# ychalier/transflow

Hardware: AMD Instinct MI355X
Metric: frames/sec (Farneback+remap) (higher is better)
Workload: dtype f32; 1 GPU; 4k: one clip of T=256 3840x2160 uint8 frames sharded over the ranks (rank r owns pairs shard_range(255, r, 1) + a one-frame halo), Farneback pyr_scale=0.5 levels=5 winsize=15 iterations=3 poly_n=5 poly_sigma=1.2 flags=0, BACKWARD post_process, moveref layer (reset random p=0.5 through a float mask, u drawn on the GPU), 1 RGB pixmap source, render; clip_frames=256, equal_batches=False

## Files before the change

### transflow_amd/csrc/common.h

```cpp
#pragma once
#include <hip/hip_runtime.h>

#include <cstdarg>
#include <cstdint>
#include <cstdio>
#include <cstdlib>
#include <string>
#include <vector>

#include "../../include/tfhip.h"

#define TF_API extern "C" __attribute__((visibility("default")))

namespace tf {

int set_error(int code, const char *fmt, ...) __attribute__((format(printf, 2, 3)));
hipStream_t stream();
hipStream_t main_stream();
int side_stream(int which, hipStream_t *out);
int ensure_init();

enum Opt { OPT_FB_FUSED = 0, OPT_FB_FUSE_MIN_PX, OPT_FB_NO_SHARE, OPT_FB_NO_OVERLAP, OPT_REMAP_PX, OPT_REMAP_NO_PACK, OPT_REMAP_KEEP_RGBA,
           OPT_PROF_LEVELS, OPT_FB_EXACT_SUMS, OPT_FB_CHAIN, OPT_FB_SEGS, OPT_REMAP_QUAD, OPT_JD_PAR_SUB_BYTES,
           OPT_JD_PAR_GROUP_SUBS, OPT_JD_PAR_STAGED, OPT_REMAP_LEAN, OPT_COUNT };
long option(Opt which);

#ifdef TF_EXPERIMENT
inline long tune(const char *env, long dflt)
{
    const char *v = getenv(env);
    return v ? atol(v) : dflt;
}
inline const char *tune_str(const char *env) { return getenv(env); }
#else
constexpr long tune(const char *, long dflt) { return dflt; }
constexpr const char *tune_str(const char *) { return nullptr; }
#endif

struct StreamScope {
    explicit StreamScope(hipStream_t s);
    ~StreamScope();
    hipStream_t prev;
};

#define TF_HIP(expr)                                                                              \
    do {                                                                                          \
        hipError_t _e = (expr);                                                                   \
        if (_e != hipSuccess)                                                                     \
            return tf::set_error(TF_ERR_HIP, "%s failed: %s (%s:%d)", #expr, hipGetErrorString(_e), \
                                 __FILE__, __LINE__);                                             \
    } while (0)

#define TF_TRY(expr)        \
    do {                    \
        int _rc = (expr);   \
        if (_rc != TF_OK)   \
            return _rc;     \
    } while (0)

#define TF_REQUIRE(cond, ...)                         \
    do {                                              \
        if (!(cond))                                  \
            return tf::set_error(TF_ERR_ARG, __VA_ARGS__); \
    } while (0)

struct ProfScope {
    explicit ProfScope(const char *name);
    ~ProfScope();
    const char *name;
    hipEvent_t a, b;
};
bool prof_enabled();

template <typename K, typename... Args>
inline int launch(const char *name, K kernel, dim3 grid, dim3 block, size_t smem, Args... args)
{
    if (grid.x == 0 || grid.y == 0 || grid.z == 0)
        return TF_OK;
    {
        ProfScope ps(name);
        hipLaunchKernelGGL(kernel, grid, block, smem, stream(), args...);
    }
    hipError_t e = hipGetLastError();
    if (e != hipSuccess)
        return set_error(TF_ERR_HIP, "launch %s failed: %s", name, hipGetErrorString(e));
    return TF_OK;
}

struct DevBuf {
    void *p = nullptr;
    size_t bytes = 0;
    bool borrowed = false;
    DevBuf() = default;
    DevBuf(const DevBuf &) = delete;
    DevBuf &operator=(const DevBuf &) = delete;
    ~DevBuf() { release(); }
    int alloc(size_t n);
    void borrow(void *ptr, size_t n);
    void release();
    template <typename T> T *as() const { return reinterpret_cast<T *>(p); }
};

struct PinnedBuf {
    void *p = nullptr;
    PinnedBuf() = default;
    PinnedBuf(const PinnedBuf &) = delete;
    PinnedBuf &operator=(const PinnedBuf &) = delete;
    ~PinnedBuf() { release(); }
    int alloc(size_t n);
    void release();
    template <typename T> T *as() const { return reinterpret_cast<T *>(p); }
};

struct Event {
    hipEvent_t e = nullptr;
    Event() = default;
    Event(const Event &) = delete;
    Event &operator=(const Event &) = delete;
    ~Event() { release(); }
    int create();
    void release();
    operator hipEvent_t() const { return e; }
};

inline unsigned cdiv(size_t a, size_t b) { return (unsigned)((a + b - 1) / b); }

struct FastDiv {
    uint32_t m;
    int s1, s2;
};
inline FastDiv fast_div_setup(uint32_t d)
{
    int s = 0;
    while ((1ull << s) < d)
        s++;
    FastDiv f;
    f.m = (uint32_t)(((1ull << 32) * ((1ull << s) - d)) / d + 1);
    f.s1 = s < 1 ? s : 1;
    f.s2 = s > 1 ? s - 1 : 0;
    return f;
}
__device__ __forceinline__ uint32_t fast_div(uint32_t t, FastDiv f)
{
    const uint32_t hi = __umulhi(t, f.m);
    return (((t - hi) >> f.s1) + hi) >> f.s2;
}

__device__ __forceinline__ float clip_nan(float v, float lo, float hi) { return v != v ? v : fminf(fmaxf(v, lo), hi); }

__device__ __forceinline__ int clampi(int v, int lo, int hi) { return v < lo ? lo : (v > hi ? hi : v); }

struct PpLabels {
    const char *clip, *fwd_scatter, *fwd_resolve, *ops;
};
constexpr PpLabels PP_FB{"pp_clip", "pp_fwd_scatter", "pp_fwd_resolve", "pp_ops"};
constexpr PpLabels PP_FLOW{"flow_pp_clip", "flow_pp_fwd_scatter", "flow_pp_fwd_resolve", "flow_pp_ops"};
int pp_ops(float2 *flow, int W, int H, int n_ops, const tf_flow_op *ops, const float *mask_dev, const PpLabels &lb);
int pp_scatter(const float2 *flow, int W, int H, int *winner, const PpLabels &lb);
int pp_direction(void *flow, bool wide, int W, int H, int direction, int *winner, const PpLabels &lb);

}
```

### transflow_amd/csrc/fb_pyramid.hip

```cpp
#include "fb_common.h"

namespace {

#ifndef TF_PX_TH
#define TF_PX_TH 16
#endif
constexpr int PX_TW = 64, PX_TH = TF_PX_TH;

__global__ void k_polyexp(const float *__restrict__ img, float *__restrict__ R, int Wk, int Hk, PolyConst pc)
{
    extern __shared__ float s_mem[];
    const int n = pc.n;
    const int LW = PX_TW + 2 * n;
    const int LH = PX_TH + 2 * n;
    float *sI = s_mem;
    float *sT = s_mem + LH * LW;
    const int pi = blockIdx.z;
    const size_t Nk = (size_t)Wk * Hk;
    const float *src = img + (size_t)pi * Nk;
    const int x0 = blockIdx.x * PX_TW, y0 = blockIdx.y * PX_TH;
    for (int idx = threadIdx.x; idx < LH * LW; idx += blockDim.x) {
        int ry = idx / LW, cx = idx % LW;
        int y = clampi(y0 - n + ry, 0, Hk - 1), x = clampi(x0 - n + cx, 0, Wk - 1);
        sI[idx] = src[(size_t)y * Wk + x];
    }
    __syncthreads();
    for (int idx = threadIdx.x; idx < PX_TH * LW; idx += blockDim.x) {
        int ty = idx / LW, cx = idx % LW;
        int y = y0 + ty;
        const float c = sI[(ty + n) * LW + cx];
        float t0 = c * pc.g[0], t1 = 0.f, t2 = 0.f;
        for (int k = 1; k <= n; k++) {
            int ya = max(y - k, 0), yb = min(y + k, Hk - 1);
            float a = sI[(ya - y0 + n) * LW + cx];
            float b = sI[(yb - y0 + n) * LW + cx];
            float p = a + b;
            t0 = t0 + pc.g[k] * p;
            t1 = t1 + pc.xg[k] * (b - a);
            t2 = t2 + pc.xxg[k] * p;
        }
        if (y >= Hk) {
            t0 = t1 = t2 = 0.f;
        }
        sT[(0 * PX_TH + ty) * LW + cx] = t0;
        sT[(1 * PX_TH + ty) * LW + cx] = t1;
        sT[(2 * PX_TH + ty) * LW + cx] = t2;
    }
    __syncthreads();
    float *dst = R + (size_t)pi * 5 * Nk;
    for (int idx = threadIdx.x; idx < PX_TH * PX_TW; idx += blockDim.x) {
        int ty = idx / PX_TW, cx = idx % PX_TW;
        int x = x0 + cx, y = y0 + ty;
        if (x >= Wk || y >= Hk)
            continue;
        const float *T0 = sT + (0 * PX_TH + ty) * LW + cx + n;
        const float *T1 = sT + (1 * PX_TH + ty) * LW + cx + n;
        const float *T2 = sT + (2 * PX_TH + ty) * LW + cx + n;
        float g0 = pc.g[0];
        double b1 = T0[0] * g0, b2 = 0, b3 = T1[0] * g0, b4 = 0, b5 = T2[0] * g0, b6 = 0;
        for (int k = 1; k <= n; k++) {
            double tg = T0[k] + T0[-k];
            g0 = pc.g[k];
            b1 = __builtin_fma(tg, (double)g0, b1);
            b4 = __builtin_fma(tg, (double)pc.xxg[k], b4);
            b2 += (T0[k] - T0[-k]) * pc.xg[k];
            b3 += (T1[k] + T1[-k]) * g0;
            b6 += (T1[k] - T1[-k]) * pc.xg[k];
            b5 += (T2[k] + T2[-k]) * g0;
        }
        size_t o = (size_t)y * Wk + x;
        const float v[5] = {(float)(b3 * pc.ig11), (float)(b2 * pc.ig11), (float)(b1 * pc.ig03 + b5 * pc.ig33),
                            (float)(b1 * pc.ig03 + b4 * pc.ig33), (float)(b6 * pc.ig55)};
        r_store_px(dst, Nk, o, v);
    }
}

typedef float float2w __attribute__((ext_vector_type(2), aligned(4)));

template <int N>
__device__ __forceinline__ void polyexp_vertical4(const f32x2 (&v)[4 + 2 * N], const PolyConst &pc, float *T0, float *T1,
                                                  float *T2, int LW)
{
#pragma unroll
    for (int q = 0; q < 4; q++) {
        const f32x2 c = v[q + N];
        f32x2 t0 = c * pc.g[0], t1 = {0.f, 0.f}, t2 = {0.f, 0.f};
#pragma unroll
        for (int k = 1; k <= N; k++) {
            const f32x2 a = v[q + N - k], b = v[q + N + k];
            const f32x2 p = a + b;
            t0 = t0 + pc.g[k] * p;
            t1 = t1 + pc.xg[k] * (b - a);
            t2 = t2 + pc.xxg[k] * p;
        }
        *reinterpret_cast<f32x2 *>(T0 + q * LW) = t0;
        *reinterpret_cast<f32x2 *>(T1 + q * LW) = t1;
        *reinterpret_cast<f32x2 *>(T2 + q * LW) = t2;
    }
}

template <int N>
__global__ void __launch_bounds__(256)
k_polyexp_t(const float *__restrict__ img, float *__restrict__ R, int Wk, int Hk, PolyConst pc)
{
    constexpr int TW = PX_TW, TH = PX_TH, LW = TW + 2 * N, LH = TH + 2 * N;
    __shared__ float sI[LH * LW];
    __shared__ float sT[3][TH][LW];
    const int pi = blockIdx.z;
    const size_t Nk = (size_t)Wk * Hk;
    const float *src = img + (size_t)pi * Nk;
    const int x0 = blockIdx.x * TW, y0 = blockIdx.y * TH;
    for (int idx = threadIdx.x; idx < LH * LW; idx += 256) {
        int ry = idx / LW, cx = idx - ry * LW;
        int y = clampi(y0 - N + ry, 0, Hk - 1), x = clampi(x0 - N + cx, 0, Wk - 1);
        sI[idx] = src[(size_t)y * Wk + x];
    }
    __syncthreads();
    static_assert(LW % 2 == 0, "column pairs");
    for (int idx = threadIdx.x; idx < (TH / 4) * (LW / 2); idx += 256) {
        const int g = idx / (LW / 2), cx = 2 * (idx - g * (LW / 2));
        f32x2 v[4 + 2 * N];
#pragma unroll
        for (int j = 0; j < 4 + 2 * N; j++)
            v[j] = *reinterpret_cast<const f32x2 *>(&sI[(4 * g + j) * LW + cx]);
        polyexp_vertical4<N>(v, pc, &sT[0][4 * g][cx], &sT[1][4 * g][cx], &sT[2][4 * g][cx], LW);
    }
    __syncthreads();
    float *dst = R + (size_t)pi * 5 * Nk;
    for (int idx = threadIdx.x; idx < TH * (TW / 2); idx += 256) {
        const int ty = idx / (TW / 2), cp = idx - ty * (TW / 2);
        const int x = x0 + 2 * cp, y = y0 + ty;
        if (x >= Wk || y >= Hk)
            continue;
        float w0[2 + 2 * N], w1[2 + 2 * N], w2[2 + 2 * N];
#pragma unroll
        for (int j = 0; j < 2 + 2 * N; j++) {
            w0[j] = sT[0][ty][2 * cp + j];
            w1[j] = sT[1][ty][2 * cp + j];
            w2[j] = sT[2][ty][2 * cp + j];
        }
        float out[2][5];
#pragma unroll
        for (int q = 0; q < 2; q++) {
            const float *T0 = w0 + q + N, *T1 = w1 + q + N, *T2 = w2 + q + N;
            float g0 = pc.g[0];
            double b1 = T0[0] * g0, b2 = 0, b3 = T1[0] * g0, b4 = 0, b5 = T2[0] * g0, b6 = 0;
#pragma unroll
            for (int k = 1; k <= N; k++) {
                double tg = T0[k] + T0[-k];
                g0 = pc.g[k];
                b1 = __builtin_fma(tg, (double)g0, b1);
                b4 = __builtin_fma(tg, (double)pc.xxg[k], b4);
                b2 += (T0[k] - T0[-k]) * pc.xg[k];
                b3 += (T1[k] + T1[-k]) * g0;
                b6 += (T1[k] - T1[-k]) * pc.xg[k];
                b5 += (T2[k] + T2[-k]) * g0;
            }
            out[q][0] = (float)(b3 * pc.ig11);
            out[q][1] = (float)(b2 * pc.ig11);
            out[q][2] = (float)(b1 * pc.ig03 + b5 * pc.ig33);
            out[q][3] = (float)(b1 * pc.ig03 + b4 * pc.ig33);
            out[q][4] = (float)(b6 * pc.ig55);
        }
        const size_t o = (size_t)y * Wk + x;
        if (x + 1 < Wk)
            r_store_px2(dst, Nk, o, out[0], out[1]);
        else
            r_store_px(dst, Nk, o, out[0]);
    }
}

template <int N, int TW, int TH>
__device__ __forceinline__ void tile_expansion(const float *sI, float (*sT)[TH][TW + 2 * N], int x0, int y0, int xr0,
                                               int yr0, int W, int H, const PolyConst &pc, float *dst, size_t Nk)
{
    constexpr int LW = TW + 2 * N;
    const bool interior = x0 - N >= 0 && x0 + TW - 1 + N <= W - 1 && y0 - N >= 0 && y0 + TH - 1 + N <= H - 1;
    for (int idx = threadIdx.x; idx < (TH / 4) * (LW / 2); idx += 256) {
        const int g = idx / (LW / 2), cx = 2 * (idx - g * (LW / 2));
        f32x2 v[4 + 2 * N];
        if (interior) {
#pragma unroll
            for (int j = 0; j < 4 + 2 * N; j++)
                v[j] = *reinterpret_cast<const f32x2 *>(&sI[(4 * g + j) * LW + cx]);
        } else {
            const int xa = clampi(x0 - N + cx, 0, W - 1) - xr0, xb = clampi(x0 - N + cx + 1, 0, W - 1) - xr0;
#pragma unroll
            for (int j = 0; j < 4 + 2 * N; j++) {
                const float *row = sI + (clampi(y0 - N + 4 * g + j, 0, H - 1) - yr0) * LW;
                v[j] = f32x2{row[xa], row[xb]};
            }
        }
        polyexp_vertical4<N>(v, pc, &sT[0][4 * g][cx], &sT[1][4 * g][cx], &sT[2][4 * g][cx], LW);
    }
    __syncthreads();
    for (int idx = threadIdx.x; idx < TH * (TW / 2); idx += 256) {
        const int ty = idx / (TW / 2), cp = idx - ty * (TW / 2);
        const int x = x0 + 2 * cp, y = y0 + ty;
        if (x >= W || y >= H)
            continue;
        float w0[2 + 2 * N], w1[2 + 2 * N], w2[2 + 2 * N];
#pragma unroll
        for (int j = 0; j < 2 + 2 * N; j++) {
            w0[j] = sT[0][ty][2 * cp + j];
            w1[j] = sT[1][ty][2 * cp + j];
            w2[j] = sT[2][ty][2 * cp + j];
        }
        float out[2][5];
#pragma unroll
        for (int q = 0; q < 2; q++) {
            const float *T0 = w0 + q + N, *T1 = w1 + q + N, *T2 = w2 + q + N;
            float g0 = pc.g[0];
            double b1 = T0[0] * g0, b2 = 0, b3 = T1[0] * g0, b4 = 0, b5 = T2[0] * g0, b6 = 0;
#pragma unroll
            for (int k = 1; k <= N; k++) {
                double tg = T0[k] + T0[-k];
                g0 = pc.g[k];
                b1 = __builtin_fma(tg, (double)g0, b1);
                b4 = __builtin_fma(tg, (double)pc.xxg[k], b4);
                b2 += (T0[k] - T0[-k]) * pc.xg[k];
                b3 += (T1[k] + T1[-k]) * g0;
                b6 += (T1[k] - T1[-k]) * pc.xg[k];
                b5 += (T2[k] + T2[-k]) * g0;
            }
            out[q][0] = (float)(b3 * pc.ig11);
            out[q][1] = (float)(b2 * pc.ig11);
            out[q][2] = (float)(b1 * pc.ig03 + b5 * pc.ig33);
            out[q][3] = (float)(b1 * pc.ig03 + b4 * pc.ig33);
            out[q][4] = (float)(b6 * pc.ig55);
        }
        const size_t o = (size_t)y * W + x;
        if (x + 1 < W)
            r_store_px2(dst, Nk, o, out[0], out[1]);
        else
            r_store_px(dst, Nk, o, out[0]);
    }
}

#ifndef TF_EXP_TH0
#define TF_EXP_TH0 16
#endif
#ifndef TF_EXP_TH1
#define TF_EXP_TH1 24
#endif
template <int N>
__global__ void __launch_bounds__(256)
k_level0_polyexp_t(const uint8_t *__restrict__ frames, const int2 *__restrict__ pairs, float *__restrict__ R, int W,
                   int H, float kc, float k1, PolyConst pc)
{
    constexpr int TW = 64, TH = TF_EXP_TH0, LW = TW + 2 * N, LH = TH + 2 * N;
    constexpr int SW = ((LW + 2 + 3 + 3) + 3) & ~3, SH = LH + 2;
    constexpr int RS = (LW + 3) & ~3;
    static_assert(SW >= RS + 4 + 4 && (SH * SW) % 16 == 0, "a group's three dwords stay inside its staged row; sRow 16-byte aligned");
    constexpr int BYTES_A = SH * SW + SH * RS * 4, BYTES_T = 3 * TH * LW * 4;
    constexpr int BYTES_U = ((BYTES_A > BYTES_T ? BYTES_A : BYTES_T) + 15) & ~15;
    __shared__ __attribute__((aligned(16))) uint8_t s_u[BYTES_U];
    __shared__ float sI[LH * LW];
    uint8_t *sS = s_u;
    float *sRow = reinterpret_cast<float *>(s_u + SH * SW);
    float(*sT)[TH][LW] = reinterpret_cast<float(*)[TH][LW]>(s_u);
    const int pi = blockIdx.z;
    const int2 pr = pairs[pi >> 1];
    const uint8_t *src = frames + (size_t)((pi & 1) ? pr.y : pr.x) * W * H;
    const size_t Nk = (size_t)W * H;
    const int x0 = blockIdx.x * TW, y0 = blockIdx.y * TH;
    const int lane = threadIdx.x & 63, wave = threadIdx.x >> 6;
    const int xr0 = max(x0 - N, 0), xr1 = min(x0 + TW - 1 + N, W - 1);
    const int yr0 = max(y0 - N, 0), yr1 = min(y0 + TH - 1 + N, H - 1);
    const int ny = yr1 - yr0 + 1;
    const int xs = (xr0 - 1) & ~3, off = xr0 - 1 - xs;
    const int ncols = xr1 + 1 - xs + 1;
    const bool dwords = (W & 3) == 0 && xs >= 0 && xs + ((ncols + 3) & ~3) <= W;
    constexpr int U = 8;
    if (dwords) {
        const int nq = (ncols + 3) >> 2;
        for (int c = lane; c < nq; c += 64) {
            for (int j0 = wave; j0 < ny + 2; j0 += 4 * U) {
                uint32_t v[U];
#pragma unroll
                for (int u = 0; u < U; u++) {
                    int ry = j0 + 4 * u;
                    if (ry < ny + 2)
                        v[u] = *reinterpret_cast<const uint32_t *>(src + (size_t)reflect101_near(yr0 - 1 + ry, H) * W + xs + 4 * c);
                }
#pragma unroll
                for (int u = 0; u < U; u++) {
                    int ry = j0 + 4 * u;
                    if (ry < ny + 2)
                        *reinterpret_cast<uint32_t *>(sS + ry * SW + 4 * c) = v[u];
                }
            }
        }
    } else {
        for (int c = lane; c < ncols; c += 64) {
            const int x = reflect101_near(xs + c, W);
            for (int j0 = wave; j0 < ny + 2; j0 += 4 * U) {
                uint8_t v[U];
#pragma unroll
                for (int u = 0; u < U; u++) {
                    int ry = j0 + 4 * u;
                    if (ry < ny + 2)
                        v[u] = src[(size_t)reflect101_near(yr0 - 1 + ry, H) * W + x];
                }
#pragma unroll
                for (int u = 0; u < U; u++) {
                    int ry = j0 + 4 * u;
                    if (ry < ny + 2)
                        sS[ry * SW + c] = v[u];
                }
            }
        }
    }
    __syncthreads();
    for (int idx = threadIdx.x; idx < (ny + 2) * (RS / 4); idx += 256) {
        const int ry = idx / (RS / 4), cx = 4 * (idx - ry * (RS / 4));
        const uint32_t *q = reinterpret_cast<const uint32_t *>(sS + ry * SW + cx);
        const uint32_t d0 = q[0], d1 = q[1], d2 = q[2];
        const uint32_t lo = __builtin_amdgcn_alignbyte(d1, d0, off), hi = __builtin_amdgcn_alignbyte(d2, d1, off);
        const float b0 = (float)(lo & 0xff), b1 = (float)((lo >> 8) & 0xff), b2 = (float)((lo >> 16) & 0xff),
                    b3 = (float)(lo >> 24), b4 = (float)(hi & 0xff), b5 = (float)((hi >> 8) & 0xff);
        float *o = sRow + ry * RS + cx;
        *reinterpret_cast<f32x2 *>(o) = f32x2{b1 * kc + (b0 + b2) * k1, b2 * kc + (b1 + b3) * k1};
        *reinterpret_cast<f32x2 *>(o + 2) = f32x2{b3 * kc + (b2 + b4) * k1, b4 * kc + (b3 + b5) * k1};
    }
    __syncthreads();
    for (int idx = threadIdx.x; idx < ny * (RS / 4); idx += 256) {
        const int ry = idx / (RS / 4), cx = 4 * (idx - ry * (RS / 4));
        const float *c = sRow + (ry + 1) * RS + cx;
        const f32x4 m = *reinterpret_cast<const f32x4 *>(c), dn = *reinterpret_cast<const f32x4 *>(c + RS),
                    up = *reinterpret_cast<const f32x4 *>(c - RS);
        f32x4 v = kc * m;
        v += k1 * (dn + up);
        float *o = sI + ry * LW + cx;
        *reinterpret_cast<f32x2 *>(o) = f32x2{v.x, v.y};
        if (cx + 2 < LW)
            *reinterpret_cast<f32x2 *>(o + 2) = f32x2{v.z, v.w};
    }
    __syncthreads();
    tile_expansion<N, TW, TH>(sI, sT, x0, y0, xr0, yr0, W, H, pc, R + (size_t)pi * 5 * Nk, Nk);
}

template <int N>
__global__ void __launch_bounds__(256)
k_level1_polyexp_t(const uint8_t *__restrict__ frames, const int2 *__restrict__ pairs, float *__restrict__ R, int W,
                   int H, float kc, float k1, PolyConst pc)
{
    constexpr int TW = 64, TH = TF_EXP_TH1, LW = TW + 2 * N, LH = TH + 2 * N;
    constexpr int SW = ((2 * LW + 2 + 3 + 3) + 3) & ~3, SH = 2 * LH + 2;
    constexpr int BYTES_A = SH * SW, BYTES_T = 3 * TH * LW * 4;
    constexpr int BYTES_U = ((BYTES_A > BYTES_T ? BYTES_A : BYTES_T) + 15) & ~15;
    __shared__ __attribute__((aligned(16))) uint8_t s_u[BYTES_U];
    __shared__ float sI[LH * LW];
    uint8_t *sS = s_u;
    float(*sT)[TH][LW] = reinterpret_cast<float(*)[TH][LW]>(s_u);
    const int Wk = W >> 1, Hk = H >> 1;
    const int pi = blockIdx.z;
    const int2 pr = pairs[pi >> 1];
    const uint8_t *src = frames + (size_t)((pi & 1) ? pr.y : pr.x) * W * H;
    const size_t Nk = (size_t)Wk * Hk;
    const int x0 = blockIdx.x * TW, y0 = blockIdx.y * TH;
    const int lane = threadIdx.x & 63, wave = threadIdx.x >> 6;
    const int xr0 = max(x0 - N, 0), xr1 = min(x0 + TW - 1 + N, Wk - 1);
    const int yr0 = max(y0 - N, 0), yr1 = min(y0 + TH - 1 + N, Hk - 1);
    const int ny = yr1 - yr0 + 1;
    const int cfirst = 2 * xr0 - 1, rfirst = 2 * yr0 - 1, nrows = 2 * ny + 2;
    const int xs = cfirst >= 0 ? (cfirst & ~3) : cfirst, off = cfirst - xs;
    const int ncols = 2 * xr1 + 2 - xs + 1;
    const bool dwords = (W & 3) == 0 && xs >= 0 && (xs & 3) == 0 && xs + ((ncols + 3) & ~3) <= W;
    constexpr int U = 8;
    if (dwords) {
        const int nq = (ncols + 3) >> 2;
        for (int c = lane; c < nq; c += 64) {
            for (int j0 = wave; j0 < nrows; j0 += 4 * U) {
                uint32_t v[U];
#pragma unroll
                for (int u = 0; u < U; u++) {
                    int ry = j0 + 4 * u;
                    if (ry < nrows)
                        v[u] = *reinterpret_cast<const uint32_t *>(src + (size_t)reflect101_near(rfirst + ry, H) * W + xs + 4 * c);
                }
#pragma unroll
                for (int u = 0; u < U; u++) {
                    int ry = j0 + 4 * u;
                    if (ry < nrows)
                        *reinterpret_cast<uint32_t *>(sS + ry * SW + 4 * c) = v[u];
                }
            }
        }
    } else {
        for (int c = lane; c < ncols; c += 64) {
            const int x = reflect101_near(xs + c, W);
            for (int j0 = wave; j0 < nrows; j0 += 4 * U) {
                uint8_t v[U];
#pragma unroll
                for (int u = 0; u < U; u++) {
                    int ry = j0 + 4 * u;
                    if (ry < nrows)
                        v[u] = src[(size_t)reflect101_near(rfirst + ry, H) * W + x];
                }
#pragma unroll
                for (int u = 0; u < U; u++) {
                    int ry = j0 + 4 * u;
                    if (ry < nrows)
                        sS[ry * SW + c] = v[u];
                }
            }
        }
    }
    __syncthreads();
    static_assert(LW % 2 == 0 && SW >= 2 * LW + 8, "2 x 2 blocks; a block's three dwords stay inside its staged row");
    for (int idx = threadIdx.x; idx < ((ny + 1) >> 1) * (LW / 2); idx += 256) {
        const int by2 = idx / (LW / 2), ry = 2 * by2, cx = 2 * (idx - by2 * (LW / 2));
        float rp[6][4];
#pragma unroll
        for (int dy = 0; dy < 6; dy++) {
            const uint32_t *q = reinterpret_cast<const uint32_t *>(sS + (2 * ry + dy) * SW + 2 * cx);
            const uint32_t d0 = q[0], d1 = q[1], d2 = q[2];
            const uint32_t lo = __builtin_amdgcn_alignbyte(d1, d0, off), hi = __builtin_amdgcn_alignbyte(d2, d1, off);
            const float b0 = (float)(lo & 0xff), b1 = (float)((lo >> 8) & 0xff), b2 = (float)((lo >> 16) & 0xff),
                        b3 = (float)(lo >> 24), b4 = (float)(hi & 0xff), b5 = (float)((hi >> 8) & 0xff);
            rp[dy][0] = b1 * kc + (b0 + b2) * k1;
            rp[dy][1] = b2 * kc + (b1 + b3) * k1;
            rp[dy][2] = b3 * kc + (b2 + b4) * k1;
            rp[dy][3] = b4 * kc + (b3 + b5) * k1;
        }
#pragma unroll
        for (int a = 0; a < 2; a++) {
            float out[2];
#pragma unroll
            for (int b = 0; b < 2; b++) {
                float v00 = kc * rp[2 * a + 1][2 * b], v01 = kc * rp[2 * a + 1][2 * b + 1];
                float v10 = kc * rp[2 * a + 2][2 * b], v11 = kc * rp[2 * a + 2][2 * b + 1];
                v00 += k1 * (rp[2 * a + 2][2 * b] + rp[2 * a][2 * b]);
                v01 += k1 * (rp[2 * a + 2][2 * b + 1] + rp[2 * a][2 * b + 1]);
                v10 += k1 * (rp[2 * a + 3][2 * b] + rp[2 * a + 1][2 * b]);
                v11 += k1 * (rp[2 * a + 3][2 * b + 1] + rp[2 * a + 1][2 * b + 1]);
                const float h0 = v00 * (1.f - 0.5f) + v01 * 0.5f, h1 = v10 * (1.f - 0.5f) + v11 * 0.5f;
                out[b] = h0 * (1.f - 0.5f) + h1 * 0.5f;
            }
            if (ry + a < ny)
                *reinterpret_cast<f32x2 *>(sI + (ry + a) * LW + cx) = f32x2{out[0], out[1]};
        }
    }
    __syncthreads();
    tile_expansion<N, TW, TH>(sI, sT, x0, y0, xr0, yr0, Wk, Hk, pc, R + (size_t)pi * 5 * Nk, Nk);
}

}

namespace tf {
namespace fb {

int fb_polyexp(tf_fb *fb, int w, int h, const ImageRun &run, int k)
{
    const int n = fb->pc.n;
    dim3 grid(cdiv(w, PX_TW), cdiv(h, PX_TH), run.n);
    if (n == 5)
        return launch(lvl_name("fb_polyexp", k), k_polyexp_t<5>, grid, dim3(256), 0, (const float *)fb->imgk(k),
                      fb->Rk(k, run), w, h, fb->pc);
    if (n == 7)
        return launch(lvl_name("fb_polyexp", k), k_polyexp_t<7>, grid, dim3(256), 0, (const float *)fb->imgk(k),
                      fb->Rk(k, run), w, h, fb->pc);
    size_t smem = ((size_t)(PX_TH + 2 * n) * (PX_TW + 2 * n) + 3 * (size_t)PX_TH * (PX_TW + 2 * n)) * sizeof(float);
    return launch(lvl_name("fb_polyexp_generic", k), k_polyexp, grid, dim3(256), smem,
                  (const float *)fb->imgk(k), fb->Rk(k, run), w, h, fb->pc);
}

static bool fb_can_fuse_level(tf_fb *fb, int k)
{
    static const bool off = tune("TF_FB_NO_A1A2", 0) != 0;
    const Level &L = *fb->lv[k];
    return !off && L.W == fb->W && L.H == fb->H && L.ksz == 3 && (fb->pc.n == 5 || fb->pc.n == 7);
}

static bool fb_can_fuse_half_level(tf_fb *fb, int k)
{
    static const bool off = tune("TF_FB_NO_A1A2", 0) != 0;
    const Level &L = *fb->lv[k];
    return !off && 2 * L.W == fb->W && 2 * L.H == fb->H && L.ksz == 3 && (fb->pc.n == 5 || fb->pc.n == 7);
}

static int fb_level1_polyexp(tf_fb *fb, int k, const ImageRun &run)
{
    Level &L = *fb->lv[k];
    dim3 grid(cdiv(L.W, 64), cdiv(L.H, TF_EXP_TH1), run.n);
    const float kc = L.kern_host[1], k1 = L.kern_host[2];
    if (fb->pc.n == 5)
        return launch(lvl_name("fb_level_polyexp", k), k_level1_polyexp_t<5>, grid, dim3(256), 0,
                      (const uint8_t *)fb->frames.as<uint8_t>(), fb->image_list(run), fb->Rk(k, run), fb->W,
                      fb->H, kc, k1, fb->pc);
    return launch(lvl_name("fb_level_polyexp", k), k_level1_polyexp_t<7>, grid, dim3(256), 0,
                  (const uint8_t *)fb->frames.as<uint8_t>(), fb->image_list(run), fb->Rk(k, run), fb->W, fb->H,
                  kc, k1, fb->pc);
}

static int fb_level0_polyexp(tf_fb *fb, int k, const ImageRun &run)
{
    Level &L = *fb->lv[k];
    dim3 grid(cdiv(L.W, 64), cdiv(L.H, TF_EXP_TH0), run.n);
    const float kc = L.kern_host[1], k1 = L.kern_host[2];
    if (fb->pc.n == 5)
        return launch(lvl_name("fb_level_polyexp", k), k_level0_polyexp_t<5>, grid, dim3(256), 0,
                      (const uint8_t *)fb->frames.as<uint8_t>(), fb->image_list(run), fb->Rk(k, run),
                      L.W, L.H, kc, k1, fb->pc);
    return launch(lvl_name("fb_level_polyexp", k), k_level0_polyexp_t<7>, grid, dim3(256), 0,
                  (const uint8_t *)fb->frames.as<uint8_t>(), fb->image_list(run), fb->Rk(k, run), L.W,
                  L.H, kc, k1, fb->pc);
}

int fb_expand_level(tf_fb *fb, int k, const ImageRun &run, bool standalone)
{
    if (fb_can_fuse_level(fb, k))
        return fb_level0_polyexp(fb, k, run);
    if (fb_can_fuse_half_level(fb, k))
        return fb_level1_polyexp(fb, k, run);
    TF_TRY(fb_level_image(fb, k, run, standalone));
    return fb_polyexp(fb, fb->lv[k]->W, fb->lv[k]->H, run, k);
}

}
}
```

### transflow_amd/csrc/runtime.hip

```cpp
#include <cstring>
#include <map>
#include <mutex>

#include "common.h"

#include <cstdlib>

namespace tf {

static thread_local std::string g_last_error;
static std::mutex g_mu;
static bool g_inited = false;
static int g_device = 0;
static hipStream_t g_stream = nullptr;

int set_error(int code, const char *fmt, ...)
{
    char buf[1024];
    va_list ap;
    va_start(ap, fmt);
    vsnprintf(buf, sizeof(buf), fmt, ap);
    va_end(ap);
    g_last_error = buf;
    return code;
}

struct OptDef {
    const char *name;
    long value, lo, hi;
};
static OptDef g_opts[OPT_COUNT] = {
    {"fb_fused", -1, -1, 1},
    {"fb_fuse_min_px", 4000000, 0, 1l << 40},
    {"fb_no_share", 0, 0, 1},
    {"fb_no_overlap", 0, 0, 1},
    {"remap_px", 4, 1, 4},
    {"remap_no_pack", 0, 0, 2},
    {"remap_keep_rgba", 0, 0, 1},
    {"prof_levels", 0, 0, 1},
    {"fb_exact_sums", 0, 0, 1},
    {"fb_chain", -1, -1, 1},
    {"fb_segs", 0, 0, 64},
    {"remap_quad", 1, 0, 1},
    {"jd_par_sub_bytes", 0, 0, 1024},
    {"jd_par_group_subs", 0, 0, 256},
    {"jd_par_staged", 0, 0, 1},
    {"remap_lean", 1, 0, 1},
};
long option(Opt which) { return g_opts[which].value; }

static thread_local hipStream_t g_override = nullptr;
static thread_local hipStream_t g_thread_main = nullptr;
static hipStream_t g_thread_streams[3] = {nullptr, nullptr, nullptr};

hipStream_t main_stream() { return g_thread_main ? g_thread_main : g_stream; }
hipStream_t stream() { return g_override ? g_override : main_stream(); }

static hipStream_t g_side[5] = {nullptr, nullptr, nullptr, nullptr, nullptr};
int side_stream(int which, hipStream_t *out)
{
    TF_REQUIRE(which >= 0 && which <= 4, "side_stream: bad index");
    TF_TRY(ensure_init());
    std::lock_guard<std::mutex> lk(g_mu);
    if (!g_side[which]) {
        int least = 0, greatest = 0;
        TF_HIP(hipDeviceGetStreamPriorityRange(&least, &greatest));
        TF_HIP(hipStreamCreateWithPriority(&g_side[which], hipStreamNonBlocking, (which == 0 || which >= 3) ? least : greatest));
    }
    *out = g_side[which];
    return TF_OK;
}

StreamScope::StreamScope(hipStream_t s) : prev(g_override) { g_override = s; }
StreamScope::~StreamScope() { g_override = prev; }

static int init_device(int device)
{
    std::lock_guard<std::mutex> lk(g_mu);
    if (g_inited) {
        if (device != g_device)
            return set_error(TF_ERR_STATE, "tf_init(%d): library already bound to device %d", device, g_device);
        TF_HIP(hipSetDevice(g_device));
        return TF_OK;
    }
    int n = 0;
    TF_HIP(hipGetDeviceCount(&n));
    if (device < 0 || device >= n)
        return set_error(TF_ERR_ARG, "tf_init: device %d out of range (%d visible)", device, n);
    TF_HIP(hipSetDevice(device));
    hipDeviceProp_t prop;
    TF_HIP(hipGetDeviceProperties(&prop, device));
    if (strncmp(prop.gcnArchName, "gfx950", 6) != 0)
        return set_error(TF_ERR_UNSUPPORTED, "tf_init: device %d is %s; this library is built for gfx950 only",
                         device, prop.gcnArchName);
    {
        int least = 0, greatest = 0;
        TF_HIP(hipDeviceGetStreamPriorityRange(&least, &greatest));
        TF_HIP(hipStreamCreateWithPriority(&g_stream, hipStreamNonBlocking, greatest));
    }
    g_device = device;
    g_inited = true;
    return TF_OK;
}

int ensure_init()
{
    if (g_inited)
        return hipSetDevice(g_device) == hipSuccess ? TF_OK : set_error(TF_ERR_HIP, "hipSetDevice failed");
    return init_device(0);
}

int DevBuf::alloc(size_t n)
{
    release();
    if (n == 0)
        return TF_OK;
    TF_HIP(hipMalloc(&p, n));
    bytes = n;
    return TF_OK;
}

void DevBuf::borrow(void *ptr, size_t n)
{
    release();
    p = ptr;
    bytes = n;
    borrowed = true;
}

void DevBuf::release()
{
    if (p && !borrowed)
        (void)hipFree(p);
    p = nullptr;
    bytes = 0;
    borrowed = false;
}

int PinnedBuf::alloc(size_t n)
{
    release();
    TF_HIP(hipHostMalloc(&p, n, hipHostMallocDefault));
    return TF_OK;
}

void PinnedBuf::release()
{
    if (p)
        (void)hipHostFree(p);
    p = nullptr;
}

int Event::create()
{
    release();
    TF_HIP(hipEventCreateWithFlags(&e, hipEventDisableTiming));
    return TF_OK;
}

void Event::release()
{
    if (e)
        (void)hipEventDestroy(e);
    e = nullptr;
}

struct ProfRec {
    const char *name;
    hipEvent_t a, b;
};
static bool g_prof = false;
static std::mutex g_prof_mu;
static std::string g_prof_filter;
static std::vector<ProfRec> g_recs;
static std::vector<hipEvent_t> g_free_events;
static std::map<std::string, std::pair<long, double>> g_acc;

bool prof_enabled() { return g_prof; }

static hipEvent_t get_event_locked()
{
    if (!g_free_events.empty()) {
        hipEvent_t e = g_free_events.back();
        g_free_events.pop_back();
        return e;
    }
    hipEvent_t e;
    (void)hipEventCreate(&e);
    return e;
}

static void prof_drain_locked()
{
    if (g_recs.empty())
        return;
    (void)hipDeviceSynchronize();
    for (auto &r : g_recs) {
        float ms = 0;
        (void)hipEventElapsedTime(&ms, r.a, r.b);
        auto &acc = g_acc[r.name];
        acc.first += 1;
        acc.second += ms;
        g_free_events.push_back(r.a);
        g_free_events.push_back(r.b);
    }
    g_recs.clear();
}

ProfScope::ProfScope(const char *name_) : name(name_), a(nullptr), b(nullptr)
{
    if (!g_prof)
        return;
    {
        std::lock_guard<std::mutex> lk(g_prof_mu);
        if (!g_prof_filter.empty() && !strstr(name, g_prof_filter.c_str()))
            return;
        if (g_recs.size() >= 4096)
            prof_drain_locked();
        a = get_event_locked();
        b = get_event_locked();
    }
    (void)hipEventRecord(a, stream());
}

ProfScope::~ProfScope()
{
    if (!a)
        return;
    (void)hipEventRecord(b, stream());
    std::lock_guard<std::mutex> lk(g_prof_mu);
    g_recs.push_back(ProfRec{name, a, b});
}

}

using namespace tf;

struct tf_event {
    hipEvent_t ev;
};

TF_API int tf_abi_version(void) { return TFHIP_ABI_VERSION; }

TF_API int tf_init(int device) { return init_device(device); }

TF_API int tf_set_option(const char *name, long value)
{
    TF_REQUIRE(name, "tf_set_option: null name");
    for (auto &o : g_opts)
        if (strcmp(o.name, name) == 0) {
            TF_REQUIRE(value >= o.lo && value <= o.hi, "tf_set_option: %s takes %ld..%ld, got %ld", name, o.lo, o.hi, value);
            o.value = value;
            return TF_OK;
        }
    return set_error(TF_ERR_ARG, "tf_set_option: unknown option '%s'", name);
}

TF_API int tf_get_option(const char *name, long *value)
{
    TF_REQUIRE(name && value, "tf_get_option: null argument");
    for (auto &o : g_opts)
        if (strcmp(o.name, name) == 0) {
            *value = o.value;
            return TF_OK;
        }
    return set_error(TF_ERR_ARG, "tf_get_option: unknown option '%s'", name);
}

TF_API int tf_is_initialized(void) { return g_inited ? 1 : 0; }

TF_API int tf_device_count(int *count)
{
    TF_REQUIRE(count, "tf_device_count: null pointer");
    TF_HIP(hipGetDeviceCount(count));
    return TF_OK;
}

TF_API const char *tf_last_error(void) { return g_last_error.c_str(); }

TF_API int tf_sync(void)
{
    TF_TRY(ensure_init());
    TF_HIP(hipStreamSynchronize(stream()));
    return TF_OK;
}

TF_API int tf_stream(void **hip_stream)
{
    TF_REQUIRE(hip_stream, "tf_stream: null pointer");
    TF_TRY(ensure_init());
    *hip_stream = (void *)stream();
    return TF_OK;
}

TF_API int tf_event_create(tf_event **ev)
{
    TF_REQUIRE(ev, "tf_event_create: null pointer");
    TF_TRY(ensure_init());
    tf_event *e = new tf_event;
    hipError_t rc = hipEventCreate(&e->ev);
    if (rc != hipSuccess) {
        delete e;
        return set_error(TF_ERR_HIP, "hipEventCreate failed: %s", hipGetErrorString(rc));
    }
    *ev = e;
    return TF_OK;
}

TF_API int tf_event_record(tf_event *ev)
{
    TF_REQUIRE(ev, "tf_event_record: null event");
    TF_HIP(hipEventRecord(ev->ev, stream()));
    return TF_OK;
}

TF_API int tf_event_elapsed_ms(tf_event *start, tf_event *stop, float *ms)
{
    TF_REQUIRE(start && stop && ms, "tf_event_elapsed_ms: null argument");
    TF_HIP(hipEventSynchronize(stop->ev));
    TF_HIP(hipEventElapsedTime(ms, start->ev, stop->ev));
    return TF_OK;
}

TF_API int tf_stream_wait_event(tf_event *ev)
{
    TF_REQUIRE(ev, "tf_stream_wait_event: null event");
    TF_TRY(ensure_init());
    TF_HIP(hipStreamWaitEvent(stream(), ev->ev, 0));
    return TF_OK;
}

TF_API int tf_event_synchronize(tf_event *ev)
{
    TF_REQUIRE(ev, "tf_event_synchronize: null event");
    TF_HIP(hipEventSynchronize(ev->ev));
    return TF_OK;
}

static_assert(sizeof(hipIpcMemHandle_t) == TF_IPC_HANDLE_BYTES, "tfhip.h states the size of an IPC handle");

TF_API int tf_ipc_export(void *dev, void *handle_out)
{
    TF_REQUIRE(dev && handle_out, "tf_ipc_export: null pointer");
    TF_TRY(ensure_init());
    hipIpcMemHandle_t h;
    TF_HIP(hipIpcGetMemHandle(&h, dev));
    memcpy(handle_out, &h, sizeof(h));
    return TF_OK;
}

TF_API int tf_ipc_open(const void *handle, void **dev)
{
    TF_REQUIRE(handle && dev, "tf_ipc_open: null pointer");
    TF_TRY(ensure_init());
    hipIpcMemHandle_t h;
    memcpy(&h, handle, sizeof(h));
    TF_HIP(hipIpcOpenMemHandle(dev, h, hipIpcMemLazyEnablePeerAccess));
    return TF_OK;
}

TF_API int tf_ipc_close(void *dev)
{
    if (dev)
        TF_HIP(hipIpcCloseMemHandle(dev));
    return TF_OK;
}

TF_API void tf_event_destroy(tf_event *ev)
{
    if (!ev)
        return;
    (void)hipEventDestroy(ev->ev);
    delete ev;
}

TF_API int tf_prof_enable(int on)
{
    TF_TRY(ensure_init());
    std::lock_guard<std::mutex> lk(g_prof_mu);
    if (!on)
        prof_drain_locked();
    g_prof = on != 0;
    return TF_OK;
}

TF_API int tf_prof_set_filter(const char *substring)
{
    std::lock_guard<std::mutex> lk(g_prof_mu);
    g_prof_filter = substring ? substring : "";
    return TF_OK;
}

TF_API int tf_prof_reset(void)
{
    std::lock_guard<std::mutex> lk(g_prof_mu);
    prof_drain_locked();
    g_acc.clear();
    return TF_OK;
}

TF_API int tf_prof_report(char *buf, size_t buf_size)
{
    TF_REQUIRE(buf && buf_size > 0, "tf_prof_report: null buffer");
    std::lock_guard<std::mutex> lk(g_prof_mu);
    prof_drain_locked();
    size_t off = 0;
    buf[0] = 0;
    for (auto &kv : g_acc) {
        int n = snprintf(buf + off, buf_size - off, "%s %ld %.6f\n", kv.first.c_str(), kv.second.first,
                         kv.second.second);
        if (n < 0 || (size_t)n >= buf_size - off)
            return set_error(TF_ERR_ARG, "tf_prof_report: buffer too small");
        off += (size_t)n;
    }
    return TF_OK;
}

TF_API int tf_thread_stream(int which)
{
    TF_REQUIRE(which >= 0 && which <= 3, "tf_thread_stream: stream %d not in 0..3", which);
    TF_TRY(ensure_init());
    if (which == 0) {
        g_thread_main = nullptr;
        return TF_OK;
    }
    {
        std::lock_guard<std::mutex> lk(g_mu);
        if (!g_thread_streams[which - 1]) {
            int least = 0, greatest = 0;
            TF_HIP(hipDeviceGetStreamPriorityRange(&least, &greatest));
            TF_HIP(hipStreamCreateWithPriority(&g_thread_streams[which - 1], hipStreamNonBlocking, greatest));
        }
    }
    g_thread_main = g_thread_streams[which - 1];
    return TF_OK;
}

TF_API int tf_host_alloc(void **host, size_t bytes)
{
    TF_REQUIRE(host, "tf_host_alloc: null pointer");
    TF_TRY(ensure_init());
    TF_HIP(hipHostMalloc(host, bytes ? bytes : 1, hipHostMallocDefault));
    return TF_OK;
}

TF_API int tf_host_free(void *host)
{
    if (host)
        TF_HIP(hipHostFree(host));
    return TF_OK;
}

TF_API int tf_dev_alloc(void **dev, size_t bytes)
{
    TF_REQUIRE(dev, "tf_dev_alloc: null pointer");
    TF_TRY(ensure_init());
    TF_HIP(hipMalloc(dev, bytes ? bytes : 1));
    return TF_OK;
}

TF_API int tf_dev_free(void *dev)
{
    if (dev)
        TF_HIP(hipFree(dev));
    return TF_OK;
}

TF_API int tf_dev_upload(void *dev, const void *host, size_t bytes)
{
    TF_REQUIRE(dev && host, "tf_dev_upload: null pointer");
    TF_TRY(ensure_init());
    TF_HIP(hipMemcpyAsync(dev, host, bytes, hipMemcpyHostToDevice, stream()));
    TF_HIP(hipStreamSynchronize(stream()));
    return TF_OK;
}

TF_API int tf_dev_download(void *host, const void *dev, size_t bytes)
{
    TF_REQUIRE(dev && host, "tf_dev_download: null pointer");
    TF_TRY(ensure_init());
    TF_HIP(hipMemcpyAsync(host, dev, bytes, hipMemcpyDeviceToHost, stream()));
    TF_HIP(hipStreamSynchronize(stream()));
    return TF_OK;
}

__global__ void k_stream_copy(const float4 *__restrict__ src, float4 *__restrict__ dst, size_t n)
{
    size_t i = (size_t)blockIdx.x * blockDim.x + threadIdx.x;
    if (i < n)
        dst[i] = src[i];
}

TF_API int tf_dev_stream_copy(void *dst_dev, const void *src_dev, size_t bytes)
{
    TF_REQUIRE(dst_dev && src_dev && (bytes & 15) == 0, "tf_dev_stream_copy: null pointer or size not a multiple of 16");
    TF_TRY(ensure_init());
    const size_t n = bytes / 16;
    return tf::launch("stream_copy", k_stream_copy, dim3(tf::cdiv(n, 256)), dim3(256), 0, (const float4 *)src_dev,
                      (float4 *)dst_dev, n);
}

__global__ void k_store_u64(unsigned long long *dst, unsigned long long v)
{
    *dst = v;
}

TF_API int tf_dev_store_u64(void *dev, uint64_t value)
{
    TF_REQUIRE(dev && ((uintptr_t)dev & 7) == 0, "tf_dev_store_u64: null or misaligned pointer");
    TF_TRY(ensure_init());
    return tf::launch("store_u64", k_store_u64, dim3(1), dim3(1), 0, (unsigned long long *)dev, (unsigned long long)value);
}

TF_API int tf_dev_copy(void *dst_dev, const void *src_dev, size_t bytes)
{
    TF_REQUIRE(dst_dev && src_dev, "tf_dev_copy: null pointer");
    TF_TRY(ensure_init());
    TF_HIP(hipMemcpyAsync(dst_dev, src_dev, bytes, hipMemcpyDeviceToDevice, stream()));
    return TF_OK;
}
```

Before: 2155 frames/s.

## Add lean polyexp path with integer 1-2-1 blur and strip-reused level-1 downsample

Result: no change. 2171 frames/s (median of 6 runs) (+0.7%).

```diff
diff --git a/transflow_amd/csrc/common.h b/transflow_amd/csrc/common.h
--- a/transflow_amd/csrc/common.h
+++ b/transflow_amd/csrc/common.h
@@ -22,7 +22,7 @@
 
 enum Opt { OPT_FB_FUSED = 0, OPT_FB_FUSE_MIN_PX, OPT_FB_NO_SHARE, OPT_FB_NO_OVERLAP, OPT_REMAP_PX, OPT_REMAP_NO_PACK, OPT_REMAP_KEEP_RGBA,
            OPT_PROF_LEVELS, OPT_FB_EXACT_SUMS, OPT_FB_CHAIN, OPT_FB_SEGS, OPT_REMAP_QUAD, OPT_JD_PAR_SUB_BYTES,
-           OPT_JD_PAR_GROUP_SUBS, OPT_JD_PAR_STAGED, OPT_REMAP_LEAN, OPT_COUNT };
+           OPT_JD_PAR_GROUP_SUBS, OPT_JD_PAR_STAGED, OPT_REMAP_LEAN, OPT_FB_EXP_LEAN, OPT_COUNT };
 long option(Opt which);
 
 #ifdef TF_EXPERIMENT
diff --git a/transflow_amd/csrc/fb_pyramid.hip b/transflow_amd/csrc/fb_pyramid.hip
--- a/transflow_amd/csrc/fb_pyramid.hip
+++ b/transflow_amd/csrc/fb_pyramid.hip
@@ -76,8 +76,9 @@
 }
 
 typedef float float2w __attribute__((ext_vector_type(2), aligned(4)));
-
-template <int N>
+typedef uint32_t u32x2 __attribute__((ext_vector_type(2)));
+
+template <int N, bool LEAN = false>
 __device__ __forceinline__ void polyexp_vertical4(const f32x2 (&v)[4 + 2 * N], const PolyConst &pc, float *T0, float *T1,
                                                   float *T2, int LW)
 {
@@ -90,8 +91,13 @@
             const f32x2 a = v[q + N - k], b = v[q + N + k];
             const f32x2 p = a + b;
             t0 = t0 + pc.g[k] * p;
-            t1 = t1 + pc.xg[k] * (b - a);
-            t2 = t2 + pc.xxg[k] * p;
+            if (LEAN && k == 1) {
+                t1 = pc.xg[k] * (b - a);
+                t2 = pc.xxg[k] * p;
+            } else {
+                t1 = t1 + pc.xg[k] * (b - a);
+                t2 = t2 + pc.xxg[k] * p;
+            }
         }
         *reinterpret_cast<f32x2 *>(T0 + q * LW) = t0;
         *reinterpret_cast<f32x2 *>(T1 + q * LW) = t1;
@@ -170,7 +176,7 @@
     }
 }
 
-template <int N, int TW, int TH>
+template <int N, int TW, int TH, bool LEAN>
 __device__ __forceinline__ void tile_expansion(const float *sI, float (*sT)[TH][TW + 2 * N], int x0, int y0, int xr0,
                                                int yr0, int W, int H, const PolyConst &pc, float *dst, size_t Nk)
 {
@@ -191,7 +197,7 @@
                 v[j] = f32x2{row[xa], row[xb]};
             }
         }
-        polyexp_vertical4<N>(v, pc, &sT[0][4 * g][cx], &sT[1][4 * g][cx], &sT[2][4 * g][cx], LW);
+        polyexp_vertical4<N, LEAN>(v, pc, &sT[0][4 * g][cx], &sT[1][4 * g][cx], &sT[2][4 * g][cx], LW);
     }
     __syncthreads();
     for (int idx = threadIdx.x; idx < TH * (TW / 2); idx += 256) {
@@ -217,10 +223,16 @@
                 double tg = T0[k] + T0[-k];
                 g0 = pc.g[k];
                 b1 = __builtin_fma(tg, (double)g0, b1);
-                b4 = __builtin_fma(tg, (double)pc.xxg[k], b4);
-                b2 += (T0[k] - T0[-k]) * pc.xg[k];
+                if (LEAN && k == 1) {
+                    b4 = tg * (double)pc.xxg[k];
+                    b2 = (T0[k] - T0[-k]) * pc.xg[k];
+                    b6 = (T1[k] - T1[-k]) * pc.xg[k];
+                } else {
+                    b4 = __builtin_fma(tg, (double)pc.xxg[k], b4);
+                    b2 += (T0[k] - T0[-k]) * pc.xg[k];
+                    b6 += (T1[k] - T1[-k]) * pc.xg[k];
+                }
                 b3 += (T1[k] + T1[-k]) * g0;
-                b6 += (T1[k] - T1[-k]) * pc.xg[k];
                 b5 += (T2[k] + T2[-k]) * g0;
             }
             out[q][0] = (float)(b3 * pc.ig11);
@@ -243,7 +255,7 @@
 #ifndef TF_EXP_TH1
 #define TF_EXP_TH1 24
 #endif
-template <int N>
+template <int N, bool LEAN>
 __global__ void __launch_bounds__(256)
 k_level0_polyexp_t(const uint8_t *__restrict__ frames, const int2 *__restrict__ pairs, float *__restrict__ R, int W,
                    int H, float kc, float k1, PolyConst pc)
@@ -252,12 +264,13 @@
     constexpr int SW = ((LW + 2 + 3 + 3) + 3) & ~3, SH = LH + 2;
     constexpr int RS = (LW + 3) & ~3;
     static_assert(SW >= RS + 4 + 4 && (SH * SW) % 16 == 0, "a group's three dwords stay inside its staged row; sRow 16-byte aligned");
-    constexpr int BYTES_A = SH * SW + SH * RS * 4, BYTES_T = 3 * TH * LW * 4;
+    constexpr int BYTES_A = SH * SW + SH * RS * (LEAN ? 2 : 4), BYTES_T = 3 * TH * LW * 4;
     constexpr int BYTES_U = ((BYTES_A > BYTES_T ? BYTES_A : BYTES_T) + 15) & ~15;
     __shared__ __attribute__((aligned(16))) uint8_t s_u[BYTES_U];
     __shared__ float sI[LH * LW];
     uint8_t *sS = s_u;
     float *sRow = reinterpret_cast<float *>(s_u + SH * SW);
+    uint16_t *sRowI = reinterpret_cast<uint16_t *>(s_u + SH * SW);
     float(*sT)[TH][LW] = reinterpret_cast<float(*)[TH][LW]>(s_u);
     const int pi = blockIdx.z;
     const int2 pr = pairs[pi >> 1];
@@ -317,6 +330,13 @@
         const uint32_t *q = reinterpret_cast<const uint32_t *>(sS + ry * SW + cx);
         const uint32_t d0 = q[0], d1 = q[1], d2 = q[2];
         const uint32_t lo = __builtin_amdgcn_alignbyte(d1, d0, off), hi = __builtin_amdgcn_alignbyte(d2, d1, off);
+        if (LEAN) {
+            const uint32_t mid = __builtin_amdgcn_alignbyte(hi, lo, 2);
+            const uint32_t r0 = __builtin_amdgcn_udot4(lo, 0x00010201u, 0u, false), r1 = __builtin_amdgcn_udot4(lo, 0x01020100u, 0u, false),
+                           r2 = __builtin_amdgcn_udot4(mid, 0x00010201u, 0u, false), r3 = __builtin_amdgcn_udot4(mid, 0x01020100u, 0u, false);
+            *reinterpret_cast<u32x2 *>(sRowI + ry * RS + cx) = u32x2{r0 | (r1 << 16), r2 | (r3 << 16)};
+            continue;
+        }
         const float b0 = (float)(lo & 0xff), b1 = (float)((lo >> 8) & 0xff), b2 = (float)((lo >> 16) & 0xff),
                     b3 = (float)(lo >> 24), b4 = (float)(hi & 0xff), b5 = (float)((hi >> 8) & 0xff);
         float *o = sRow + ry * RS + cx;
@@ -326,21 +346,30 @@
     __syncthreads();
     for (int idx = threadIdx.x; idx < ny * (RS / 4); idx += 256) {
         const int ry = idx / (RS / 4), cx = 4 * (idx - ry * (RS / 4));
-        const float *c = sRow + (ry + 1) * RS + cx;
-        const f32x4 m = *reinterpret_cast<const f32x4 *>(c), dn = *reinterpret_cast<const f32x4 *>(c + RS),
-                    up = *reinterpret_cast<const f32x4 *>(c - RS);
-        f32x4 v = kc * m;
-        v += k1 * (dn + up);
+        f32x4 v;
+        if (LEAN) {
+            const uint16_t *c = sRowI + (ry + 1) * RS + cx;
+            const u32x2 m = *reinterpret_cast<const u32x2 *>(c), dn = *reinterpret_cast<const u32x2 *>(c + RS),
+                        up = *reinterpret_cast<const u32x2 *>(c - RS);
+            const u32x2 s = up + 2u * m + dn;
+            v = f32x4{(float)(s.x & 0xffffu), (float)(s.x >> 16), (float)(s.y & 0xffffu), (float)(s.y >> 16)} * 0.0625f;
+        } else {
+            const float *c = sRow + (ry + 1) * RS + cx;
+            const f32x4 m = *reinterpret_cast<const f32x4 *>(c), dn = *reinterpret_cast<const f32x4 *>(c + RS),
+                        up = *reinterpret_cast<const f32x4 *>(c - RS);
+            v = kc * m;
+            v += k1 * (dn + up);
+        }
         float *o = sI + ry * LW + cx;
         *reinterpret_cast<f32x2 *>(o) = f32x2{v.x, v.y};
         if (cx + 2 < LW)
             *reinterpret_cast<f32x2 *>(o + 2) = f32x2{v.z, v.w};
     }
     __syncthreads();
-    tile_expansion<N, TW, TH>(sI, sT, x0, y0, xr0, yr0, W, H, pc, R + (size_t)pi * 5 * Nk, Nk);
-}
-
-template <int N>
+    tile_expansion<N, TW, TH, LEAN>(sI, sT, x0, y0, xr0, yr0, W, H, pc, R + (size_t)pi * 5 * Nk, Nk);
+}
+
+template <int N, bool LEAN>
 __global__ void __launch_bounds__(256)
 k_level1_polyexp_t(const uint8_t *__restrict__ frames, const int2 *__restrict__ pairs, float *__restrict__ R, int W,
                    int H, float kc, float k1, PolyConst pc)
@@ -409,7 +438,50 @@
     }
     __syncthreads();
     static_assert(LW % 2 == 0 && SW >= 2 * LW + 8, "2 x 2 blocks; a block's three dwords stay inside its staged row");
-    for (int idx = threadIdx.x; idx < ((ny + 1) >> 1) * (LW / 2); idx += 256) {
+    constexpr int L1 = 7, STRIPS = (LH + L1 - 1) / L1;
+    static_assert((2 * STRIPS * L1 + 2) * SW <= BYTES_U, "the last strip's reads stay inside s_u");
+    for (int idx = threadIdx.x; LEAN && idx < ((ny + L1 - 1) / L1) * (LW / 2); idx += 256) {
+        const int st = idx / (LW / 2), ry = L1 * st, cx = 2 * (idx - st * (LW / 2));
+        float ra[4], rb[4];
+        auto rowpass = [&](int srow, float(&rp)[4]) {
+            const uint32_t *q = reinterpret_cast<const uint32_t *>(sS + srow * SW + 2 * cx);
+            const uint32_t d0 = q[0], d1 = q[1], d2 = q[2];
+            const uint32_t lo = __builtin_amdgcn_alignbyte(d1, d0, off), hi = __builtin_amdgcn_alignbyte(d2, d1, off);
+            const float b0 = (float)(lo & 0xff), b1 = (float)((lo >> 8) & 0xff), b2 = (float)((lo >> 16) & 0xff),
+                        b3 = (float)(lo >> 24), b4 = (float)(hi & 0xff), b5 = (float)((hi >> 8) & 0xff);
+            rp[0] = b1 * kc + (b0 + b2) * k1;
+            rp[1] = b2 * kc + (b1 + b3) * k1;
+            rp[2] = b3 * kc + (b2 + b4) * k1;
+            rp[3] = b4 * kc + (b3 + b5) * k1;
+        };
+        rowpass(2 * ry, ra);
+        rowpass(2 * ry + 1, rb);
+#pragma unroll
+        for (int a = 0; a < L1; a++) {
+            float rc[4], rd[4];
+            rowpass(2 * (ry + a) + 2, rc);
+            rowpass(2 * (ry + a) + 3, rd);
+            float out[2];
+#pragma unroll
+            for (int b = 0; b < 2; b++) {
+                float v00 = kc * rb[2 * b], v01 = kc * rb[2 * b + 1];
+                float v10 = kc * rc[2 * b], v11 = kc * rc[2 * b + 1];
+                v00 += k1 * (rc[2 * b] + ra[2 * b]);
+                v01 += k1 * (rc[2 * b + 1] + ra[2 * b + 1]);
+                v10 += k1 * (rd[2 * b] + rb[2 * b]);
+                v11 += k1 * (rd[2 * b + 1] + rb[2 * b + 1]);
+                out[b] = ((v00 + v01) + (v10 + v11)) * 0.25f;
+            }
+            if (ry + a < ny)
+                *reinterpret_cast<f32x2 *>(sI + (ry + a) * LW + cx) = f32x2{out[0], out[1]};
+#pragma unroll
+            for (int j = 0; j < 4; j++) {
+                ra[j] = rc[j];
+                rb[j] = rd[j];
+            }
+        }
+    }
+    for (int idx = threadIdx.x; !LEAN && idx < ((ny + 1) >> 1) * (LW / 2); idx += 256) {
         const int by2 = idx / (LW / 2), ry = 2 * by2, cx = 2 * (idx - by2 * (LW / 2));
         float rp[6][4];
 #pragma unroll
@@ -443,7 +515,7 @@
         }
     }
     __syncthreads();
-    tile_expansion<N, TW, TH>(sI, sT, x0, y0, xr0, yr0, Wk, Hk, pc, R + (size_t)pi * 5 * Nk, Nk);
+    tile_expansion<N, TW, TH, LEAN>(sI, sT, x0, y0, xr0, yr0, Wk, Hk, pc, R + (size_t)pi * 5 * Nk, Nk);
 }
 
 }
@@ -480,18 +552,23 @@
     return !off && 2 * L.W == fb->W && 2 * L.H == fb->H && L.ksz == 3 && (fb->pc.n == 5 || fb->pc.n == 7);
 }
 
+static bool fb_exp_lean(const tf_fb *fb, float kc, float k1)
+{
+    const float least = 0x1p-40f;
+    return option(OPT_FB_EXP_LEAN) == 1 && kc >= least && k1 >= least && fb->pc.g[1] >= least && fb->pc.xg[1] >= least &&
+           fb->pc.xxg[1] >= least;
+}
+
 static int fb_level1_polyexp(tf_fb *fb, int k, const ImageRun &run)
 {
     Level &L = *fb->lv[k];
     dim3 grid(cdiv(L.W, 64), cdiv(L.H, TF_EXP_TH1), run.n);
     const float kc = L.kern_host[1], k1 = L.kern_host[2];
-    if (fb->pc.n == 5)
-        return launch(lvl_name("fb_level_polyexp", k), k_level1_polyexp_t<5>, grid, dim3(256), 0,
-                      (const uint8_t *)fb->frames.as<uint8_t>(), fb->image_list(run), fb->Rk(k, run), fb->W,
-                      fb->H, kc, k1, fb->pc);
-    return launch(lvl_name("fb_level_polyexp", k), k_level1_polyexp_t<7>, grid, dim3(256), 0,
-                  (const uint8_t *)fb->frames.as<uint8_t>(), fb->image_list(run), fb->Rk(k, run), fb->W, fb->H,
-                  kc, k1, fb->pc);
+    const bool lean = fb_exp_lean(fb, kc, k1);
+    auto kernel = fb->pc.n == 5 ? (lean ? k_level1_polyexp_t<5, true> : k_level1_polyexp_t<5, false>)
+                                : (lean ? k_level1_polyexp_t<7, true> : k_level1_polyexp_t<7, false>);
+    return launch(lvl_name("fb_level_polyexp", k), kernel, grid, dim3(256), 0, (const uint8_t *)fb->frames.as<uint8_t>(),
+                  fb->image_list(run), fb->Rk(k, run), fb->W, fb->H, kc, k1, fb->pc);
 }
 
 static int fb_level0_polyexp(tf_fb *fb, int k, const ImageRun &run)
@@ -499,13 +576,11 @@
     Level &L = *fb->lv[k];
     dim3 grid(cdiv(L.W, 64), cdiv(L.H, TF_EXP_TH0), run.n);
     const float kc = L.kern_host[1], k1 = L.kern_host[2];
-    if (fb->pc.n == 5)
-        return launch(lvl_name("fb_level_polyexp", k), k_level0_polyexp_t<5>, grid, dim3(256), 0,
-                      (const uint8_t *)fb->frames.as<uint8_t>(), fb->image_list(run), fb->Rk(k, run),
-                      L.W, L.H, kc, k1, fb->pc);
-    return launch(lvl_name("fb_level_polyexp", k), k_level0_polyexp_t<7>, grid, dim3(256), 0,
-                  (const uint8_t *)fb->frames.as<uint8_t>(), fb->image_list(run), fb->Rk(k, run), L.W,
-                  L.H, kc, k1, fb->pc);
+    const bool lean = fb_exp_lean(fb, kc, k1) && kc == 0.5f && k1 == 0.25f;
+    auto kernel = fb->pc.n == 5 ? (lean ? k_level0_polyexp_t<5, true> : k_level0_polyexp_t<5, false>)
+                                : (lean ? k_level0_polyexp_t<7, true> : k_level0_polyexp_t<7, false>);
+    return launch(lvl_name("fb_level_polyexp", k), kernel, grid, dim3(256), 0, (const uint8_t *)fb->frames.as<uint8_t>(),
+                  fb->image_list(run), fb->Rk(k, run), L.W, L.H, kc, k1, fb->pc);
 }
 
 int fb_expand_level(tf_fb *fb, int k, const ImageRun &run, bool standalone)
diff --git a/transflow_amd/csrc/runtime.hip b/transflow_amd/csrc/runtime.hip
--- a/transflow_amd/csrc/runtime.hip
+++ b/transflow_amd/csrc/runtime.hip
@@ -46,6 +46,7 @@
     {"jd_par_group_subs", 0, 0, 256},
     {"jd_par_staged", 0, 0, 1},
     {"remap_lean", 1, 0, 1},
+    {"fb_exp_lean", 1, 0, 1},
 };
 long option(Opt which) { return g_opts[which].value; }
 
```
